# nyu-systems/Grendel-GS

Measured on NVIDIA H100. Metric: train-step Gaussians/s (preprocess+forward+loss+backward), higher is better.
Workload: dtype f32

## Files before the change

### grendel-gs_b200/csrc/loss.cu

```cuda
#include "common.cuh"

#define LS_TILE 32
#define LS_HALO 5
#define LS_IN (LS_TILE + 2 * LS_HALO)
#define LS_THREADS 256

__device__ __constant__ float c_gauss[11];
static unsigned long long g_gauss_ready = 0ull;

static int ensure_gauss() {
    int dev = 0;
    GS_CUDA_TRY(cudaGetDevice(&dev));
    if (dev < 64 && ((g_gauss_ready >> dev) & 1ull)) return GS_OK;
    float g[11], s = 0.f;
    for (int k = 0; k < 11; k++) { g[k] = (float)exp(-((double)(k - 5) * (k - 5)) / (2.0 * 1.5 * 1.5)); s += g[k]; }
    for (int k = 0; k < 11; k++) g[k] = g[k] / s;
    GS_CUDA_TRY(cudaMemcpyToSymbol(c_gauss, g, sizeof(g)));
    if (dev < 64) g_gauss_ready |= 1ull << dev;
    return GS_OK;
}

extern "C" size_t gs_loss_temp_bytes(int rows, int image_width) {
    return (size_t)9 * (size_t)(rows > 0 ? rows : 0) * (size_t)image_width * sizeof(float) + 256;
}

struct LossViews {
    int row0[GS_MAX_VIEWS], rows[GS_MAX_VIEWS];
    int crow0[GS_MAX_VIEWS], crow1[GS_MAX_VIEWS];
    const uint8_t *gt[GS_MAX_VIEWS];
    unsigned long long map_off[GS_MAX_VIEWS];
};

__global__ void __launch_bounds__(LS_THREADS)
k_loss_fwd(int W, int H, const LossViews lv, const float *__restrict__ image, float *__restrict__ maps,
           double *__restrict__ sums) {
    __shared__ float s_x[LS_IN][LS_IN + 1], s_y[LS_IN][LS_IN + 1];
    __shared__ float s_h[5][LS_IN][LS_TILE + 1];
    __shared__ float s_red[2][LS_THREADS / 32];
    const int view = blockIdx.z;
    const int row0 = lv.row0[view], rows = lv.rows[view], crow0 = lv.crow0[view], crow1 = lv.crow1[view];
    const int tx0 = blockIdx.x * LS_TILE, ty0 = blockIdx.y * LS_TILE;
    if (ty0 >= rows) return;
    const size_t HW = (size_t)H * W, SW = (size_t)rows * W;
    const uint8_t *__restrict__ gt = lv.gt[view];
    image += (size_t)view * 3 * HW;
    maps += lv.map_off[view];
    sums += 2 * view;
    const float C1 = 0.01f * 0.01f, C2 = 0.03f * 0.03f;
    float l1 = 0.f, ss = 0.f;
    for (int ch = 0; ch < 3; ch++) {
        for (int k = threadIdx.x; k < LS_IN * LS_IN; k += LS_THREADS) {
            const int r = k / LS_IN, c = k % LS_IN;
            const int y = ty0 + r - LS_HALO, x = tx0 + c - LS_HALO;
            float vx = 0.f, vy = 0.f;
            if (y >= 0 && y < rows && x >= 0 && x < W) {
                vx = image[ch * HW + (size_t)(row0 + y) * W + x];
                vy = fminf(1.f, fmaxf(0.f, (float)gt[ch * SW + (size_t)y * W + x] / 255.0f));
            }
            s_x[r][c] = vx; s_y[r][c] = vy;
        }
        __syncthreads();
        for (int k = threadIdx.x; k < LS_IN * (LS_TILE / 4); k += LS_THREADS) {
            const int r = k / (LS_TILE / 4), c0 = (k % (LS_TILE / 4)) * 4;
            float wx[14], wy[14];
#pragma unroll
            for (int t = 0; t < 14; t++) { wx[t] = s_x[r][c0 + t]; wy[t] = s_y[r][c0 + t]; }
#pragma unroll
            for (int q = 0; q < 4; q++) {
                float a0 = 0.f, a1 = 0.f, a2 = 0.f, a3 = 0.f, a4 = 0.f;
#pragma unroll
                for (int t = 0; t < 11; t++) {
                    const float g = c_gauss[t], vx = wx[q + t], vy = wy[q + t];
                    a0 += g * vx; a1 += g * vy; a2 += g * vx * vx; a3 += g * vy * vy; a4 += g * vx * vy;
                }
                s_h[0][r][c0 + q] = a0; s_h[1][r][c0 + q] = a1; s_h[2][r][c0 + q] = a2; s_h[3][r][c0 + q] = a3;
                s_h[4][r][c0 + q] = a4;
            }
        }
        __syncthreads();
        {
            const int c = threadIdx.x % LS_TILE, r0 = (threadIdx.x / LS_TILE) * 4, x = tx0 + c;
            float m1[4] = {0.f, 0.f, 0.f, 0.f}, m2[4] = {0.f, 0.f, 0.f, 0.f}, e11[4] = {0.f, 0.f, 0.f, 0.f},
                  e22[4] = {0.f, 0.f, 0.f, 0.f}, e12[4] = {0.f, 0.f, 0.f, 0.f};
#pragma unroll
            for (int t = 0; t < 14; t++) {
                const float v0 = s_h[0][r0 + t][c], v1 = s_h[1][r0 + t][c], v2 = s_h[2][r0 + t][c], v3 = s_h[3][r0 + t][c],
                            v4 = s_h[4][r0 + t][c];
#pragma unroll
                for (int q = 0; q < 4; q++) {
                    if (t - q >= 0 && t - q < 11) {
                        const float g = c_gauss[t - q];
                        m1[q] += g * v0; m2[q] += g * v1; e11[q] += g * v2; e22[q] += g * v3; e12[q] += g * v4;
                    }
                }
            }
#pragma unroll
            for (int q = 0; q < 4; q++) {
                const int r = r0 + q, y = ty0 + r;
                if (y < rows && x < W) {
                    const size_t o = (size_t)ch * SW + (size_t)y * W + x;
                    if (y < crow0 || y >= crow1) {
                        maps[o] = 0.f; maps[3 * SW + o] = 0.f; maps[6 * SW + o] = 0.f;
                    } else {
                        const float s1 = e11[q] - m1[q] * m1[q], s2 = e22[q] - m2[q] * m2[q], s12 = e12[q] - m1[q] * m2[q];
                        const float A = 2.f * m1[q] * m2[q] + C1, B = 2.f * s12 + C2,
                                    Cc = m1[q] * m1[q] + m2[q] * m2[q] + C1, D = s1 + s2 + C2;
                        const float iCD = 1.f / (Cc * D);
                        ss += A * B * iCD;
                        const float vx = s_x[r + LS_HALO][c + LS_HALO], vy = s_y[r + LS_HALO][c + LS_HALO];
                        l1 += fabsf(vx - vy);
                        maps[o] = 2.f * m2[q] * (B - A) * iCD - 2.f * m1[q] * A * B * (D - Cc) * iCD * iCD;
                        maps[3 * SW + o] = -A * B * iCD / D;
                        maps[6 * SW + o] = 2.f * A * iCD;
                    }
                }
            }
        }
        __syncthreads();
    }
#pragma unroll
    for (int o = 16; o > 0; o >>= 1) { l1 += __shfl_xor_sync(0xffffffffu, l1, o); ss += __shfl_xor_sync(0xffffffffu, ss, o); }
    if ((threadIdx.x & 31) == 0) { s_red[0][threadIdx.x >> 5] = l1; s_red[1][threadIdx.x >> 5] = ss; }
    __syncthreads();
    if (threadIdx.x == 0) {
        double a = 0.0, b = 0.0;
        for (int w = 0; w < LS_THREADS / 32; w++) { a += (double)s_red[0][w]; b += (double)s_red[1][w]; }
        atomicAdd(&sums[0], a); atomicAdd(&sums[1], b);
    }
}

__global__ void k_loss_finalize(int n, const double *__restrict__ sums, double inv_norm, float *__restrict__ out) {
    const int k = blockIdx.x * blockDim.x + threadIdx.x;
    if (k < 2 * n) out[k] = (float)(sums[k] * inv_norm);
}

__global__ void __launch_bounds__(LS_THREADS)
k_loss_bwd(int W, int H, const LossViews lv, const float *__restrict__ image, const float *__restrict__ maps,
           const float *__restrict__ grad_l1, const float *__restrict__ grad_ssim, float inv_norm,
           float *__restrict__ dimg) {
    __shared__ float s_m[3][LS_IN][LS_IN + 1];
    __shared__ float s_h[3][LS_IN][LS_TILE + 1];
    const int view = blockIdx.z;
    const int row0 = lv.row0[view], rows = lv.rows[view], crow0 = lv.crow0[view], crow1 = lv.crow1[view];
    const int tx0 = blockIdx.x * LS_TILE, ty0 = blockIdx.y * LS_TILE;
    if (ty0 >= rows) return;
    const size_t HW = (size_t)H * W, SW = (size_t)rows * W;
    const uint8_t *__restrict__ gt = lv.gt[view];
    image += (size_t)view * 3 * HW;
    dimg += (size_t)view * 3 * HW;
    maps += lv.map_off[view];
    const float gl1 = grad_l1[view] * inv_norm, gss = grad_ssim[view] * inv_norm;
    for (int ch = 0; ch < 3; ch++) {
        for (int k = threadIdx.x; k < LS_IN * LS_IN; k += LS_THREADS) {
            const int r = k / LS_IN, c = k % LS_IN;
            const int y = ty0 + r - LS_HALO, x = tx0 + c - LS_HALO;
            float v0 = 0.f, v1 = 0.f, v2 = 0.f;
            if (y >= 0 && y < rows && x >= 0 && x < W) {
                const size_t o = (size_t)ch * SW + (size_t)y * W + x;
                v0 = maps[o]; v1 = maps[3 * SW + o]; v2 = maps[6 * SW + o];
            }
            s_m[0][r][c] = v0; s_m[1][r][c] = v1; s_m[2][r][c] = v2;
        }
        __syncthreads();
        for (int k = threadIdx.x; k < LS_IN * (LS_TILE / 4); k += LS_THREADS) {
            const int r = k / (LS_TILE / 4), c0 = (k % (LS_TILE / 4)) * 4;
            float w0[14], w1[14], w2[14];
#pragma unroll
            for (int t = 0; t < 14; t++) { w0[t] = s_m[0][r][c0 + t]; w1[t] = s_m[1][r][c0 + t]; w2[t] = s_m[2][r][c0 + t]; }
#pragma unroll
            for (int q = 0; q < 4; q++) {
                float a0 = 0.f, a1 = 0.f, a2 = 0.f;
#pragma unroll
                for (int t = 0; t < 11; t++) {
                    const float g = c_gauss[t];
                    a0 += g * w0[q + t]; a1 += g * w1[q + t]; a2 += g * w2[q + t];
                }
                s_h[0][r][c0 + q] = a0; s_h[1][r][c0 + q] = a1; s_h[2][r][c0 + q] = a2;
            }
        }
        __syncthreads();
        {
            const int c = threadIdx.x % LS_TILE, r0 = (threadIdx.x / LS_TILE) * 4, x = tx0 + c;
            float b0[4] = {0.f, 0.f, 0.f, 0.f}, b1[4] = {0.f, 0.f, 0.f, 0.f}, b2[4] = {0.f, 0.f, 0.f, 0.f};
#pragma unroll
            for (int t = 0; t < 14; t++) {
                const float v0 = s_h[0][r0 + t][c], v1 = s_h[1][r0 + t][c], v2 = s_h[2][r0 + t][c];
#pragma unroll
                for (int q = 0; q < 4; q++) {
                    if (t - q >= 0 && t - q < 11) {
                        const float g = c_gauss[t - q];
                        b0[q] += g * v0; b1[q] += g * v1; b2[q] += g * v2;
                    }
                }
            }
#pragma unroll
            for (int q = 0; q < 4; q++) {
                const int y = ty0 + r0 + q;
                if (y < rows && x < W) {
                    const size_t oi = ch * HW + (size_t)(row0 + y) * W + x;
                    const float vx = image[oi];
                    const float vy = fminf(1.f, fmaxf(0.f, (float)gt[ch * SW + (size_t)y * W + x] / 255.0f));
                    const float d = vx - vy;
                    const float sgn = (y < crow0 || y >= crow1) ? 0.f : (d > 0.f ? 1.f : (d < 0.f ? -1.f : 0.f));
                    dimg[oi] = gl1 * sgn + gss * (b0[q] + 2.f * vx * b1[q] + vy * b2[q]);
                }
            }
        }
        __syncthreads();
    }
}

#define LS_HEADER_1 ((size_t)256)
#define LS_HEADER_B ((size_t)(2 * sizeof(double) * GS_MAX_VIEWS))

static int make_loss_views(int num_views, int H, int W, const int32_t *rows4, const void *const *gts, LossViews &lv,
                           int *max_rows, size_t *sum_rows) {
    GS_REQUIRE(num_views >= 1 && num_views <= GS_MAX_VIEWS, "num_views must be in [1, GS_MAX_VIEWS]");
    GS_REQUIRE(H > 0 && W > 0 && rows4 && gts, "sizes");
    size_t off = 0;
    int mx = 0;
    for (int v = 0; v < GS_MAX_VIEWS; v++) {
        lv.row0[v] = lv.rows[v] = lv.crow0[v] = lv.crow1[v] = 0;
        lv.gt[v] = nullptr;
        lv.map_off[v] = 0ull;
        if (v >= num_views) continue;
        const int row0 = rows4[4 * v], row1 = rows4[4 * v + 1], c0 = rows4[4 * v + 2], c1 = rows4[4 * v + 3];
        const int rows = row1 - row0;
        GS_REQUIRE(row0 >= 0 && row1 <= H && rows >= 0, "strip rows");
        if (rows == 0) continue;
        GS_REQUIRE(c0 >= row0 && c1 <= row1 && c1 >= c0, "count rows must lie inside [row0,row1)");
        GS_REQUIRE(gts[v] != nullptr, "null ground-truth pointer");
        lv.row0[v] = row0; lv.rows[v] = rows; lv.crow0[v] = c0 - row0; lv.crow1[v] = c1 - row0;
        lv.gt[v] = (const uint8_t *)gts[v];
        lv.map_off[v] = (unsigned long long)off;
        off += (size_t)9 * rows * W;
        mx = rows > mx ? rows : mx;
    }
    *max_rows = mx;
    *sum_rows = off / ((size_t)9 * W);
    return GS_OK;
}

static int loss_forward_impl(int num_views, int H, int W, const int32_t *rows4, const float *image, const void *const *gts,
                             float *out, void *temp, size_t temp_bytes, size_t header, cudaStream_t stream) {
    GS_REQUIRE(image && out && temp, "null pointer");
    LossViews lv;
    int max_rows = 0;
    size_t sum_rows = 0;
    int rc = make_loss_views(num_views, H, W, rows4, gts, lv, &max_rows, &sum_rows);
    if (rc != GS_OK) return rc;
    if (temp_bytes < header + (size_t)9 * sum_rows * W * sizeof(float)) {
        gs_set_error("gs_loss_forward: temp too small");
        return GS_ENOMEM;
    }
    rc = ensure_gauss();
    if (rc != GS_OK) return rc;
    double *sums = (double *)temp;
    float *maps = (float *)((char *)temp + header);
    GS_CUDA_TRY(cudaMemsetAsync(sums, 0, 2 * sizeof(double) * (size_t)num_views, stream));
    GsStageTimer timer(GS_STAGE_LOSS_FWD, stream);
    if (max_rows > 0) {
        dim3 grid((W + LS_TILE - 1) / LS_TILE, (max_rows + LS_TILE - 1) / LS_TILE, num_views);
        k_loss_fwd<<<grid, LS_THREADS, 0, stream>>>(W, H, lv, image, maps, sums);
        GS_LAUNCH_CHECK();
    }
    k_loss_finalize<<<1, 2 * GS_MAX_VIEWS, 0, stream>>>(num_views, sums, 1.0 / (3.0 * (double)H * (double)W), out);
    GS_LAUNCH_CHECK();
    return GS_OK;
}

static int loss_backward_impl(int num_views, int H, int W, const int32_t *rows4, const float *image,
                              const void *const *gts, const void *temp, const float *grad_l1, const float *grad_ssim,
                              float *dimg, size_t header, cudaStream_t stream) {
    GS_REQUIRE(image && temp && grad_l1 && grad_ssim && dimg, "null pointer");
    LossViews lv;
    int max_rows = 0;
    size_t sum_rows = 0;
    int rc = make_loss_views(num_views, H, W, rows4, gts, lv, &max_rows, &sum_rows);
    if (rc != GS_OK) return rc;
    rc = ensure_gauss();
    if (rc != GS_OK) return rc;
    const float *maps = (const float *)((const char *)temp + header);
    const size_t HW = (size_t)H * W;
    if (num_views == 1) {
        const int row0 = lv.row0[0], row1 = lv.row0[0] + lv.rows[0];
        for (int ch = 0; ch < 3; ch++) {
            if (row0 > 0) GS_CUDA_TRY(cudaMemsetAsync(dimg + ch * HW, 0, sizeof(float) * (size_t)row0 * W, stream));
            if (row1 < H)
                GS_CUDA_TRY(cudaMemsetAsync(dimg + ch * HW + (size_t)row1 * W, 0, sizeof(float) * (size_t)(H - row1) * W, stream));
        }
    } else if (sum_rows < (size_t)num_views * H) {
        GS_CUDA_TRY(cudaMemsetAsync(dimg, 0, sizeof(float) * 3 * HW * (size_t)num_views, stream));
    }
    if (max_rows == 0) return GS_OK;
    dim3 grid((W + LS_TILE - 1) / LS_TILE, (max_rows + LS_TILE - 1) / LS_TILE, num_views);
    GsStageTimer timer(GS_STAGE_LOSS_BWD, stream);
    k_loss_bwd<<<grid, LS_THREADS, 0, stream>>>(W, H, lv, image, maps, grad_l1, grad_ssim,
                                                (float)(1.0 / (3.0 * (double)H * (double)W)), dimg);
    GS_LAUNCH_CHECK();
    return GS_OK;
}

extern "C" int gs_loss_forward(int image_height, int image_width, int row0, int row1, int count_row0, int count_row1,
                               const float *image, const uint8_t *gt_u8, float *out_l1_ssim, void *temp,
                               size_t temp_bytes, void *stream_) {
    GS_REQUIRE(row1 > row0, "strip rows");
    GS_REQUIRE(gt_u8, "null pointer");
    const int32_t rows4[4] = {row0, row1, count_row0, count_row1};
    const void *gts[1] = {gt_u8};
    return loss_forward_impl(1, image_height, image_width, rows4, image, gts, out_l1_ssim, temp, temp_bytes, LS_HEADER_1,
                             (cudaStream_t)stream_);
}

extern "C" size_t gs_loss_temp_bytes_batched(int num_views, const int32_t *rows4_host, int image_width) {
    size_t rows = 0;
    for (int v = 0; v < num_views && rows4_host; v++) {
        const int r = rows4_host[4 * v + 1] - rows4_host[4 * v];
        rows += r > 0 ? (size_t)r : 0;
    }
    return LS_HEADER_B + (size_t)9 * rows * (size_t)(image_width > 0 ? image_width : 0) * sizeof(float) + 256;
}

extern "C" int gs_loss_forward_batched(int num_views, int image_height, int image_width, const int32_t *rows4_host,
                                       const float *image, const void *const *gt_u8_ptrs_host, float *out_l1_ssim,
                                       void *temp, size_t temp_bytes, void *stream_) {
    return loss_forward_impl(num_views, image_height, image_width, rows4_host, image, gt_u8_ptrs_host, out_l1_ssim, temp,
                             temp_bytes, LS_HEADER_B, (cudaStream_t)stream_);
}

extern "C" int gs_loss_backward(int image_height, int image_width, int row0, int row1, int count_row0, int count_row1,
                                const float *image, const uint8_t *gt_u8, const void *temp, const float *grad_l1,
                                const float *grad_ssim, float *dL_dimage, void *stream_) {
    GS_REQUIRE(row1 > row0, "strip rows");
    GS_REQUIRE(gt_u8, "null pointer");
    const int32_t rows4[4] = {row0, row1, count_row0, count_row1};
    const void *gts[1] = {gt_u8};
    return loss_backward_impl(1, image_height, image_width, rows4, image, gts, temp, grad_l1, grad_ssim, dL_dimage,
                              LS_HEADER_1, (cudaStream_t)stream_);
}

extern "C" int gs_loss_backward_batched(int num_views, int image_height, int image_width, const int32_t *rows4_host,
                                        const float *image, const void *const *gt_u8_ptrs_host, const void *temp,
                                        const float *grad_l1, const float *grad_ssim, float *dL_dimage, void *stream_) {
    return loss_backward_impl(num_views, image_height, image_width, rows4_host, image, gt_u8_ptrs_host, temp, grad_l1,
                              grad_ssim, dL_dimage, LS_HEADER_B, (cudaStream_t)stream_);
}
```

Baseline: 597.0 million.

## Restructure SSIM loss kernels into per-channel vertical strips with ring-buffered halo reuse

The forward and backward SSIM/L1 loss kernels now give each CTA one channel and a strip of up to 96 rows instead of a 32x32 tile over all three channels. Row-filtered results sit in a shared-memory ring buffer, so vertical halo rows are reused across consecutive 32-row chunks rather than recomputed per tile. Global loads for the next chunk are software-prefetched into registers while the current chunk is filtered. Blocks shrink to 128 threads with a minimum-CTA launch bound, and the row pass uses float4 shared accesses. The aim is less redundant halo loading and filtering plus better latency hiding, at the cost of more registers, fewer CTAs, and a more complex schedule. A separate profiling script times the loss kernels.

```diff
diff --git a/grendel-gs_b200/csrc/loss.cu b/grendel-gs_b200/csrc/loss.cu
--- a/grendel-gs_b200/csrc/loss.cu
+++ b/grendel-gs_b200/csrc/loss.cu
@@ -1,9 +1,15 @@
 #include "common.cuh"
 
-#define LS_TILE 32
 #define LS_HALO 5
-#define LS_IN (LS_TILE + 2 * LS_HALO)
-#define LS_THREADS 256
+#define LS_TW 32
+#define LS_IW (LS_TW + 2 * LS_HALO)
+#define LS_SP 44
+#define LS_CR 32
+#define LS_RING (LS_CR + 2 * LS_HALO)
+#define LS_STRIP (3 * LS_CR)
+#define LS_THREADS 128
+#define LS_MIN_CTAS 5
+#define LS_VR (LS_CR / (LS_THREADS / 32))
 
 __device__ __constant__ float c_gauss[11];
 static unsigned long long g_gauss_ready = 0ull;
@@ -31,101 +37,193 @@
     unsigned long long map_off[GS_MAX_VIEWS];
 };
 
-__global__ void __launch_bounds__(LS_THREADS)
+GS_D float gt_value(uint32_t v) {
+    const float f = (float)v, r = 1.0f / 255.0f;
+    const float q = __fmul_rn(f, r);
+    return __fmaf_rn(__fmaf_rn(-q, 255.0f, f), r, q);
+}
+
+#define LS_SSLOTS ((LS_CR * LS_IW + LS_THREADS - 1) / LS_THREADS)
+GS_D bool stage_slot(int m, int n, int &r, int &c) {
+    const int e = threadIdx.x + m * LS_THREADS;
+    r = e / LS_IW;
+    c = e - r * LS_IW;
+    return r < n;
+}
+
+template <int NI, int NQ>
+GS_D void row_pass(const float (*s_in)[LS_CR][LS_SP], float (*s_h)[LS_RING][LS_TW], int i0, int n) {
+    for (int k = threadIdx.x; k < n * (LS_TW / 4); k += LS_THREADS) {
+        const int r = k / (LS_TW / 4), c0 = (k % (LS_TW / 4)) * 4;
+        float w[NI][16];
+#pragma unroll
+        for (int p = 0; p < NI; p++)
+#pragma unroll
+            for (int m = 0; m < 4; m++) {
+                const float4 v = *reinterpret_cast<const float4 *>(&s_in[p][r][c0 + 4 * m]);
+                w[p][4 * m] = v.x; w[p][4 * m + 1] = v.y; w[p][4 * m + 2] = v.z; w[p][4 * m + 3] = v.w;
+            }
+        float a[NQ][4];
+#pragma unroll
+        for (int p = 0; p < NQ; p++)
+#pragma unroll
+            for (int q = 0; q < 4; q++) a[p][q] = 0.f;
+#pragma unroll
+        for (int j = 0; j < 14; j++) {
+            float v[NQ];
+#pragma unroll
+            for (int p = 0; p < NI; p++) v[p] = w[p][j];
+            if (NI == 2) { v[2] = w[0][j] * w[0][j]; v[3] = w[1][j] * w[1][j]; v[4] = w[0][j] * w[1][j]; }
+#pragma unroll
+            for (int q = 0; q < 4; q++) {
+                const int t = j - q;
+                if (t >= 0 && t < 11) {
+#pragma unroll
+                    for (int p = 0; p < NQ; p++) a[p][q] = fmaf(c_gauss[t], v[p], a[p][q]);
+                }
+            }
+        }
+        const int slot = (i0 + r) % LS_RING;
+#pragma unroll
+        for (int p = 0; p < NQ; p++)
+            *reinterpret_cast<float4 *>(&s_h[p][slot][c0]) = make_float4(a[p][0], a[p][1], a[p][2], a[p][3]);
+    }
+}
+
+template <int NQ>
+GS_D void col_pass(const float (*s_h)[LS_RING][LS_TW], int o0, float (&a)[NQ][LS_VR]) {
+    const int c = threadIdx.x % LS_TW;
+    int slot = (o0 + (threadIdx.x / 32) * LS_VR) % LS_RING;
+#pragma unroll
+    for (int p = 0; p < NQ; p++)
+#pragma unroll
+        for (int q = 0; q < LS_VR; q++) a[p][q] = 0.f;
+#pragma unroll
+    for (int j = 0; j < LS_VR + 10; j++) {
+        float v[NQ];
+#pragma unroll
+        for (int p = 0; p < NQ; p++) v[p] = s_h[p][slot][c];
+#pragma unroll
+        for (int q = 0; q < LS_VR; q++) {
+            const int t = j - q;
+            if (t >= 0 && t < 11) {
+#pragma unroll
+                for (int p = 0; p < NQ; p++) a[p][q] = fmaf(c_gauss[t], v[p], a[p][q]);
+            }
+        }
+        slot = slot == LS_RING - 1 ? 0 : slot + 1;
+    }
+}
+
+struct StripCta {
+    int view, ch, rows, sy0, span, tx0;
+    GS_D StripCta(const LossViews &lv) {
+        view = blockIdx.z;
+        ch = blockIdx.y % 3;
+        rows = lv.rows[view];
+        sy0 = (blockIdx.y / 3) * LS_STRIP;
+        span = min(LS_STRIP, rows - sy0);
+        tx0 = blockIdx.x * LS_TW;
+    }
+};
+
+template <class Load, class Store, class Row, class Col>
+GS_D void strip_schedule(int span, Load &&load, Store &&store, Row &&row, Col &&col) {
+    const int units = 1 + (span + LS_CR - 1) / LS_CR;
+    auto first = [](int u) { return u == 0 ? 0 : 2 * LS_HALO + (u - 1) * LS_CR; };
+    auto count = [span](int u) { return u == 0 ? 2 * LS_HALO : min(LS_CR, span - (u - 1) * LS_CR); };
+    load(first(0), count(0));
+    store(first(0), count(0));
+    __syncthreads();
+    for (int u = 0; u < units; u++) {
+        if (u + 1 < units) load(first(u + 1), count(u + 1));
+        row(first(u), count(u));
+        __syncthreads();
+        if (u + 1 < units) store(first(u + 1), count(u + 1));
+        if (u > 0) col((u - 1) * LS_CR, count(u));
+        __syncthreads();
+    }
+}
+
+__global__ void __launch_bounds__(LS_THREADS, LS_MIN_CTAS)
 k_loss_fwd(int W, int H, const LossViews lv, const float *__restrict__ image, float *__restrict__ maps,
            double *__restrict__ sums) {
-    __shared__ float s_x[LS_IN][LS_IN + 1], s_y[LS_IN][LS_IN + 1];
-    __shared__ float s_h[5][LS_IN][LS_TILE + 1];
+    __shared__ __align__(16) float s_in[2][LS_CR][LS_SP];
+    __shared__ __align__(16) float s_h[5][LS_RING][LS_TW];
     __shared__ float s_red[2][LS_THREADS / 32];
-    const int view = blockIdx.z;
-    const int row0 = lv.row0[view], rows = lv.rows[view], crow0 = lv.crow0[view], crow1 = lv.crow1[view];
-    const int tx0 = blockIdx.x * LS_TILE, ty0 = blockIdx.y * LS_TILE;
-    if (ty0 >= rows) return;
+    const StripCta b(lv);
+    if (b.span <= 0) return;
+    const int rows = b.rows, crow0 = max(lv.crow0[b.view], b.sy0), crow1 = min(lv.crow1[b.view], b.sy0 + b.span);
     const size_t HW = (size_t)H * W, SW = (size_t)rows * W;
-    const uint8_t *__restrict__ gt = lv.gt[view];
-    image += (size_t)view * 3 * HW;
-    maps += lv.map_off[view];
-    sums += 2 * view;
+    const float *__restrict__ xin = image + ((size_t)b.view * 3 + b.ch) * HW + (size_t)lv.row0[b.view] * W;
+    const uint8_t *__restrict__ yin = lv.gt[b.view] + b.ch * SW;
+    maps += lv.map_off[b.view] + b.ch * SW;
+    const int lane = threadIdx.x % 32, warp = threadIdx.x / 32, x = b.tx0 + lane;
     const float C1 = 0.01f * 0.01f, C2 = 0.03f * 0.03f;
     float l1 = 0.f, ss = 0.f;
-    for (int ch = 0; ch < 3; ch++) {
-        for (int k = threadIdx.x; k < LS_IN * LS_IN; k += LS_THREADS) {
-            const int r = k / LS_IN, c = k % LS_IN;
-            const int y = ty0 + r - LS_HALO, x = tx0 + c - LS_HALO;
-            float vx = 0.f, vy = 0.f;
-            if (y >= 0 && y < rows && x >= 0 && x < W) {
-                vx = image[ch * HW + (size_t)(row0 + y) * W + x];
-                vy = fminf(1.f, fmaxf(0.f, (float)gt[ch * SW + (size_t)y * W + x] / 255.0f));
-            }
-            s_x[r][c] = vx; s_y[r][c] = vy;
-        }
-        __syncthreads();
-        for (int k = threadIdx.x; k < LS_IN * (LS_TILE / 4); k += LS_THREADS) {
-            const int r = k / (LS_TILE / 4), c0 = (k % (LS_TILE / 4)) * 4;
-            float wx[14], wy[14];
-#pragma unroll
-            for (int t = 0; t < 14; t++) { wx[t] = s_x[r][c0 + t]; wy[t] = s_y[r][c0 + t]; }
-#pragma unroll
-            for (int q = 0; q < 4; q++) {
-                float a0 = 0.f, a1 = 0.f, a2 = 0.f, a3 = 0.f, a4 = 0.f;
-#pragma unroll
-                for (int t = 0; t < 11; t++) {
-                    const float g = c_gauss[t], vx = wx[q + t], vy = wy[q + t];
-                    a0 += g * vx; a1 += g * vy; a2 += g * vx * vx; a3 += g * vy * vy; a4 += g * vx * vy;
+    float vx[LS_SSLOTS];
+    uint32_t vg[LS_SSLOTS];
+    auto load = [&](int i0, int n) {
+        const int y0 = b.sy0 - LS_HALO + i0;
+        const ptrdiff_t base = (ptrdiff_t)y0 * W + (b.tx0 - LS_HALO);
+#pragma unroll
+        for (int m = 0; m < LS_SSLOTS; m++) {
+            int r, c;
+            const bool slot = stage_slot(m, n, r, c);
+            vx[m] = 0.f; vg[m] = 0u;
+            if (slot && (unsigned)(y0 + r) < (unsigned)rows && (unsigned)(b.tx0 - LS_HALO + c) < (unsigned)W) {
+                vx[m] = xin[base + r * W + c];
+                vg[m] = yin[base + r * W + c];
+            }
+        }
+    };
+    auto store = [&](int i0, int n) {
+#pragma unroll
+        for (int m = 0; m < LS_SSLOTS; m++) {
+            int r, c;
+            if (!stage_slot(m, n, r, c)) continue;
+            const float vy = gt_value(vg[m]);
+            if ((unsigned)(b.sy0 - LS_HALO + i0 + r - crow0) < (unsigned)(crow1 - crow0) &&
+                (unsigned)(c - LS_HALO) < (unsigned)min(LS_TW, W - b.tx0))
+                l1 += fabsf(vx[m] - vy);
+            s_in[0][r][c] = vx[m]; s_in[1][r][c] = vy;
+        }
+    };
+    auto row = [&](int i0, int n) { row_pass<2, 5>(s_in, s_h, i0, n); };
+    auto col = [&](int o0, int n) {
+        float a[5][LS_VR];
+        col_pass<5>(s_h, o0, a);
+        const int yb = b.sy0 + o0 + warp * LS_VR;
+        float *mp = maps + (ptrdiff_t)yb * W + x;
+#pragma unroll
+        for (int q = 0; q < LS_VR; q++) {
+            const int y = yb + q;
+            if (warp * LS_VR + q < n && x < W) {
+                const int off = q * W;
+                if (y < crow0 || y >= crow1) {
+                    mp[off] = 0.f; mp[3 * SW + off] = 0.f; mp[6 * SW + off] = 0.f;
+                } else {
+                    const float m1 = a[0][q], m2 = a[1][q];
+                    const float s1 = a[2][q] - m1 * m1, s2 = a[3][q] - m2 * m2, s12 = a[4][q] - m1 * m2;
+                    const float A = 2.f * m1 * m2 + C1, B = 2.f * s12 + C2, Cc = m1 * m1 + m2 * m2 + C1, D = s1 + s2 + C2;
+                    const float iCD = 1.f / (Cc * D);
+                    ss += A * B * iCD;
+                    mp[off] = 2.f * m2 * (B - A) * iCD - 2.f * m1 * A * B * (D - Cc) * iCD * iCD;
+                    mp[3 * SW + off] = -A * B * iCD / D;
+                    mp[6 * SW + off] = 2.f * A * iCD;
                 }
-                s_h[0][r][c0 + q] = a0; s_h[1][r][c0 + q] = a1; s_h[2][r][c0 + q] = a2; s_h[3][r][c0 + q] = a3;
-                s_h[4][r][c0 + q] = a4;
-            }
-        }
-        __syncthreads();
-        {
-            const int c = threadIdx.x % LS_TILE, r0 = (threadIdx.x / LS_TILE) * 4, x = tx0 + c;
-            float m1[4] = {0.f, 0.f, 0.f, 0.f}, m2[4] = {0.f, 0.f, 0.f, 0.f}, e11[4] = {0.f, 0.f, 0.f, 0.f},
-                  e22[4] = {0.f, 0.f, 0.f, 0.f}, e12[4] = {0.f, 0.f, 0.f, 0.f};
-#pragma unroll
-            for (int t = 0; t < 14; t++) {
-                const float v0 = s_h[0][r0 + t][c], v1 = s_h[1][r0 + t][c], v2 = s_h[2][r0 + t][c], v3 = s_h[3][r0 + t][c],
-                            v4 = s_h[4][r0 + t][c];
-#pragma unroll
-                for (int q = 0; q < 4; q++) {
-                    if (t - q >= 0 && t - q < 11) {
-                        const float g = c_gauss[t - q];
-                        m1[q] += g * v0; m2[q] += g * v1; e11[q] += g * v2; e22[q] += g * v3; e12[q] += g * v4;
-                    }
-                }
-            }
-#pragma unroll
-            for (int q = 0; q < 4; q++) {
-                const int r = r0 + q, y = ty0 + r;
-                if (y < rows && x < W) {
-                    const size_t o = (size_t)ch * SW + (size_t)y * W + x;
-                    if (y < crow0 || y >= crow1) {
-                        maps[o] = 0.f; maps[3 * SW + o] = 0.f; maps[6 * SW + o] = 0.f;
-                    } else {
-                        const float s1 = e11[q] - m1[q] * m1[q], s2 = e22[q] - m2[q] * m2[q], s12 = e12[q] - m1[q] * m2[q];
-                        const float A = 2.f * m1[q] * m2[q] + C1, B = 2.f * s12 + C2,
-                                    Cc = m1[q] * m1[q] + m2[q] * m2[q] + C1, D = s1 + s2 + C2;
-                        const float iCD = 1.f / (Cc * D);
-                        ss += A * B * iCD;
-                        const float vx = s_x[r + LS_HALO][c + LS_HALO], vy = s_y[r + LS_HALO][c + LS_HALO];
-                        l1 += fabsf(vx - vy);
-                        maps[o] = 2.f * m2[q] * (B - A) * iCD - 2.f * m1[q] * A * B * (D - Cc) * iCD * iCD;
-                        maps[3 * SW + o] = -A * B * iCD / D;
-                        maps[6 * SW + o] = 2.f * A * iCD;
-                    }
-                }
-            }
-        }
-        __syncthreads();
-    }
+            }
+        }
+    };
+    strip_schedule(b.span, load, store, row, col);
 #pragma unroll
     for (int o = 16; o > 0; o >>= 1) { l1 += __shfl_xor_sync(0xffffffffu, l1, o); ss += __shfl_xor_sync(0xffffffffu, ss, o); }
-    if ((threadIdx.x & 31) == 0) { s_red[0][threadIdx.x >> 5] = l1; s_red[1][threadIdx.x >> 5] = ss; }
+    if (lane == 0) { s_red[0][warp] = l1; s_red[1][warp] = ss; }
     __syncthreads();
     if (threadIdx.x == 0) {
-        double a = 0.0, b = 0.0;
-        for (int w = 0; w < LS_THREADS / 32; w++) { a += (double)s_red[0][w]; b += (double)s_red[1][w]; }
-        atomicAdd(&sums[0], a); atomicAdd(&sums[1], b);
+        double a = 0.0, c = 0.0;
+        for (int w = 0; w < LS_THREADS / 32; w++) { a += (double)s_red[0][w]; c += (double)s_red[1][w]; }
+        atomicAdd(&sums[2 * b.view], a); atomicAdd(&sums[2 * b.view + 1], c);
     }
 }
 
@@ -134,80 +232,69 @@
     if (k < 2 * n) out[k] = (float)(sums[k] * inv_norm);
 }
 
-__global__ void __launch_bounds__(LS_THREADS)
+__global__ void __launch_bounds__(LS_THREADS, LS_MIN_CTAS)
 k_loss_bwd(int W, int H, const LossViews lv, const float *__restrict__ image, const float *__restrict__ maps,
            const float *__restrict__ grad_l1, const float *__restrict__ grad_ssim, float inv_norm,
            float *__restrict__ dimg) {
-    __shared__ float s_m[3][LS_IN][LS_IN + 1];
-    __shared__ float s_h[3][LS_IN][LS_TILE + 1];
-    const int view = blockIdx.z;
-    const int row0 = lv.row0[view], rows = lv.rows[view], crow0 = lv.crow0[view], crow1 = lv.crow1[view];
-    const int tx0 = blockIdx.x * LS_TILE, ty0 = blockIdx.y * LS_TILE;
-    if (ty0 >= rows) return;
+    __shared__ __align__(16) float s_in[3][LS_CR][LS_SP];
+    __shared__ __align__(16) float s_h[3][LS_RING][LS_TW];
+    const StripCta b(lv);
+    if (b.span <= 0) return;
+    const int rows = b.rows, crow0 = lv.crow0[b.view], crow1 = lv.crow1[b.view];
     const size_t HW = (size_t)H * W, SW = (size_t)rows * W;
-    const uint8_t *__restrict__ gt = lv.gt[view];
-    image += (size_t)view * 3 * HW;
-    dimg += (size_t)view * 3 * HW;
-    maps += lv.map_off[view];
-    const float gl1 = grad_l1[view] * inv_norm, gss = grad_ssim[view] * inv_norm;
-    for (int ch = 0; ch < 3; ch++) {
-        for (int k = threadIdx.x; k < LS_IN * LS_IN; k += LS_THREADS) {
-            const int r = k / LS_IN, c = k % LS_IN;
-            const int y = ty0 + r - LS_HALO, x = tx0 + c - LS_HALO;
-            float v0 = 0.f, v1 = 0.f, v2 = 0.f;
-            if (y >= 0 && y < rows && x >= 0 && x < W) {
-                const size_t o = (size_t)ch * SW + (size_t)y * W + x;
-                v0 = maps[o]; v1 = maps[3 * SW + o]; v2 = maps[6 * SW + o];
-            }
-            s_m[0][r][c] = v0; s_m[1][r][c] = v1; s_m[2][r][c] = v2;
-        }
-        __syncthreads();
-        for (int k = threadIdx.x; k < LS_IN * (LS_TILE / 4); k += LS_THREADS) {
-            const int r = k / (LS_TILE / 4), c0 = (k % (LS_TILE / 4)) * 4;
-            float w0[14], w1[14], w2[14];
-#pragma unroll
-            for (int t = 0; t < 14; t++) { w0[t] = s_m[0][r][c0 + t]; w1[t] = s_m[1][r][c0 + t]; w2[t] = s_m[2][r][c0 + t]; }
-#pragma unroll
-            for (int q = 0; q < 4; q++) {
-                float a0 = 0.f, a1 = 0.f, a2 = 0.f;
-#pragma unroll
-                for (int t = 0; t < 11; t++) {
-                    const float g = c_gauss[t];
-                    a0 += g * w0[q + t]; a1 += g * w1[q + t]; a2 += g * w2[q + t];
-                }
-                s_h[0][r][c0 + q] = a0; s_h[1][r][c0 + q] = a1; s_h[2][r][c0 + q] = a2;
-            }
-        }
-        __syncthreads();
-        {
-            const int c = threadIdx.x % LS_TILE, r0 = (threadIdx.x / LS_TILE) * 4, x = tx0 + c;
-            float b0[4] = {0.f, 0.f, 0.f, 0.f}, b1[4] = {0.f, 0.f, 0.f, 0.f}, b2[4] = {0.f, 0.f, 0.f, 0.f};
-#pragma unroll
-            for (int t = 0; t < 14; t++) {
-                const float v0 = s_h[0][r0 + t][c], v1 = s_h[1][r0 + t][c], v2 = s_h[2][r0 + t][c];
-#pragma unroll
-                for (int q = 0; q < 4; q++) {
-                    if (t - q >= 0 && t - q < 11) {
-                        const float g = c_gauss[t - q];
-                        b0[q] += g * v0; b1[q] += g * v1; b2[q] += g * v2;
-                    }
-                }
-            }
-#pragma unroll
-            for (int q = 0; q < 4; q++) {
-                const int y = ty0 + r0 + q;
-                if (y < rows && x < W) {
-                    const size_t oi = ch * HW + (size_t)(row0 + y) * W + x;
-                    const float vx = image[oi];
-                    const float vy = fminf(1.f, fmaxf(0.f, (float)gt[ch * SW + (size_t)y * W + x] / 255.0f));
-                    const float d = vx - vy;
-                    const float sgn = (y < crow0 || y >= crow1) ? 0.f : (d > 0.f ? 1.f : (d < 0.f ? -1.f : 0.f));
-                    dimg[oi] = gl1 * sgn + gss * (b0[q] + 2.f * vx * b1[q] + vy * b2[q]);
-                }
-            }
-        }
-        __syncthreads();
-    }
+    const size_t plane = ((size_t)b.view * 3 + b.ch) * HW + (size_t)lv.row0[b.view] * W;
+    const float *__restrict__ xin = image + plane;
+    const uint8_t *__restrict__ yin = lv.gt[b.view] + b.ch * SW;
+    dimg += plane;
+    maps += lv.map_off[b.view] + b.ch * SW;
+    const int warp = threadIdx.x / 32, x = b.tx0 + threadIdx.x % 32;
+    const float gl1 = grad_l1[b.view] * inv_norm, gss = grad_ssim[b.view] * inv_norm;
+    float v[LS_SSLOTS][3];
+    auto load = [&](int i0, int n) {
+        const int y0 = b.sy0 - LS_HALO + i0;
+        const float *mp = maps + (ptrdiff_t)y0 * W + (b.tx0 - LS_HALO);
+#pragma unroll
+        for (int m = 0; m < LS_SSLOTS; m++) {
+            int r, c;
+            const bool slot = stage_slot(m, n, r, c);
+            v[m][0] = v[m][1] = v[m][2] = 0.f;
+            if (slot && (unsigned)(y0 + r) < (unsigned)rows && (unsigned)(b.tx0 - LS_HALO + c) < (unsigned)W) {
+                const int off = r * W + c;
+                v[m][0] = mp[off]; v[m][1] = mp[3 * SW + off]; v[m][2] = mp[6 * SW + off];
+            }
+        }
+    };
+    auto store = [&](int, int n) {
+#pragma unroll
+        for (int m = 0; m < LS_SSLOTS; m++) {
+            int r, c;
+            if (!stage_slot(m, n, r, c)) continue;
+            s_in[0][r][c] = v[m][0]; s_in[1][r][c] = v[m][1]; s_in[2][r][c] = v[m][2];
+        }
+    };
+    auto row = [&](int i0, int n) { row_pass<3, 3>(s_in, s_h, i0, n); };
+    auto col = [&](int o0, int n) {
+        const int yb = b.sy0 + o0 + warp * LS_VR;
+        const ptrdiff_t pb = (ptrdiff_t)yb * W + x;
+        float px[LS_VR], py[LS_VR];
+#pragma unroll
+        for (int q = 0; q < LS_VR; q++) {
+            px[q] = py[q] = 0.f;
+            if (warp * LS_VR + q < n && x < W) { px[q] = xin[pb + q * W]; py[q] = gt_value(yin[pb + q * W]); }
+        }
+        float a[3][LS_VR];
+        col_pass<3>(s_h, o0, a);
+#pragma unroll
+        for (int q = 0; q < LS_VR; q++) {
+            const int y = yb + q;
+            if (warp * LS_VR + q < n && x < W) {
+                const float d = px[q] - py[q];
+                const float sgn = (y < crow0 || y >= crow1) ? 0.f : (d > 0.f ? 1.f : (d < 0.f ? -1.f : 0.f));
+                dimg[pb + q * W] = gl1 * sgn + gss * (a[0][q] + 2.f * px[q] * a[1][q] + py[q] * a[2][q]);
+            }
+        }
+    };
+    strip_schedule(b.span, load, store, row, col);
 }
 
 #define LS_HEADER_1 ((size_t)256)
@@ -241,6 +328,10 @@
     return GS_OK;
 }
 
+static dim3 loss_grid(int W, int max_rows, int num_views) {
+    return dim3((W + LS_TW - 1) / LS_TW, 3 * ((max_rows + LS_STRIP - 1) / LS_STRIP), num_views);
+}
+
 static int loss_forward_impl(int num_views, int H, int W, const int32_t *rows4, const float *image, const void *const *gts,
                              float *out, void *temp, size_t temp_bytes, size_t header, cudaStream_t stream) {
     GS_REQUIRE(image && out && temp, "null pointer");
@@ -260,8 +351,7 @@
     GS_CUDA_TRY(cudaMemsetAsync(sums, 0, 2 * sizeof(double) * (size_t)num_views, stream));
     GsStageTimer timer(GS_STAGE_LOSS_FWD, stream);
     if (max_rows > 0) {
-        dim3 grid((W + LS_TILE - 1) / LS_TILE, (max_rows + LS_TILE - 1) / LS_TILE, num_views);
-        k_loss_fwd<<<grid, LS_THREADS, 0, stream>>>(W, H, lv, image, maps, sums);
+        k_loss_fwd<<<loss_grid(W, max_rows, num_views), LS_THREADS, 0, stream>>>(W, H, lv, image, maps, sums);
         GS_LAUNCH_CHECK();
     }
     k_loss_finalize<<<1, 2 * GS_MAX_VIEWS, 0, stream>>>(num_views, sums, 1.0 / (3.0 * (double)H * (double)W), out);
@@ -293,10 +383,9 @@
         GS_CUDA_TRY(cudaMemsetAsync(dimg, 0, sizeof(float) * 3 * HW * (size_t)num_views, stream));
     }
     if (max_rows == 0) return GS_OK;
-    dim3 grid((W + LS_TILE - 1) / LS_TILE, (max_rows + LS_TILE - 1) / LS_TILE, num_views);
     GsStageTimer timer(GS_STAGE_LOSS_BWD, stream);
-    k_loss_bwd<<<grid, LS_THREADS, 0, stream>>>(W, H, lv, image, maps, grad_l1, grad_ssim,
-                                                (float)(1.0 / (3.0 * (double)H * (double)W)), dimg);
+    k_loss_bwd<<<loss_grid(W, max_rows, num_views), LS_THREADS, 0, stream>>>(
+        W, H, lv, image, maps, grad_l1, grad_ssim, (float)(1.0 / (3.0 * (double)H * (double)W)), dimg);
     GS_LAUNCH_CHECK();
     return GS_OK;
 }
diff --git a/profiles/time_loss.py b/profiles/time_loss.py
--- /dev/null
+++ b/profiles/time_loss.py
@@ -0,0 +1,109 @@
+#!/usr/bin/env python
+import argparse
+import json
+import os
+import subprocess
+import sys
+
+ROOT = os.path.dirname(os.path.dirname(os.path.abspath(__file__)))
+for _p in (ROOT, os.path.join(ROOT, "grendel-gs_b200")):
+    if _p not in sys.path:
+        sys.path.insert(0, _p)
+
+FWD_BYTES, BWD_BYTES = 51, 63
+
+
+def card():
+    import torch
+    out = {"name": torch.cuda.get_device_name(0), "power_limit_w": None, "sm_clock_max_mhz": None}
+    try:
+        r = subprocess.run(["nvidia-smi", "--id=0", "--query-gpu=power.limit,clocks.max.sm", "--format=csv,noheader,nounits"],
+                           capture_output=True, text=True, timeout=30)
+        p, c = (v.strip() for v in r.stdout.strip().split(","))
+        out["power_limit_w"], out["sm_clock_max_mhz"] = float(p), float(c)
+    except Exception:
+        pass
+    return out
+
+
+def time_calls(fn, launches, warmup):
+    import torch
+    for _ in range(warmup):
+        fn()
+    torch.cuda.synchronize()
+    a, b = torch.cuda.Event(enable_timing=True), torch.cuda.Event(enable_timing=True)
+    a.record()
+    for _ in range(launches):
+        fn()
+    b.record()
+    torch.cuda.synchronize()
+    return a.elapsed_time(b) * 1e3 / launches
+
+
+def measure(H, W, rows4, launches, warmup):
+    import torch
+    from gs_b200 import _lib
+    row0, row1, c0, c1 = rows4
+    rows = row1 - row0
+    g = torch.Generator(device="cuda").manual_seed(0)
+    image = torch.rand((3, H, W), generator=g, device="cuda", dtype=torch.float32)
+    gt = torch.randint(0, 256, (3, rows, W), generator=g, device="cuda", dtype=torch.uint8)
+    tb = _lib.query("gs_loss_temp_bytes", rows, W)
+    temp = torch.empty((tb,), dtype=torch.uint8, device="cuda")
+    out = torch.empty((2,), dtype=torch.float32, device="cuda")
+    gw = torch.tensor([0.8, -0.2], dtype=torch.float32, device="cuda")
+    dimg = torch.empty_like(image)
+    s = torch.cuda.current_stream().cuda_stream
+
+    def fwd():
+        _lib.call("gs_loss_forward", H, W, row0, row1, c0, c1, image.data_ptr(), gt.data_ptr(), out.data_ptr(),
+                  temp.data_ptr(), tb, s)
+
+    def bwd():
+        _lib.call("gs_loss_backward", H, W, row0, row1, c0, c1, image.data_ptr(), gt.data_ptr(), temp.data_ptr(),
+                  gw.data_ptr(), gw.data_ptr() + 4, dimg.data_ptr(), s)
+
+    fwd()
+    res = {"shape": f"{W}x{H}", "rows": [row0, row1], "count_rows": [c0, c1], "launches": launches, "warmup": warmup}
+    for name, fn, per_px in (("forward", fwd, FWD_BYTES), ("backward", bwd, BWD_BYTES)):
+        us = time_calls(fn, launches, warmup)
+        _lib.profile_enable(True)
+        for _ in range(launches):
+            fn()
+        torch.cuda.synchronize()
+        stages = _lib.profile_read()
+        _lib.profile_enable(False)
+        st = stages.get("loss " + name)
+        kernel_us = st[0] * 1e3 / st[1] if st else None
+        nbytes = per_px * rows * W
+        res[name] = {"us_per_call": round(us, 2), "us_stage_timer": None if kernel_us is None else round(kernel_us, 2),
+                     "compulsory_bytes": nbytes, "gbs_per_call": round(nbytes / (us * 1e-6) / 1e9, 1),
+                     "frac_of_3350_gbs": round(nbytes / (us * 1e-6) / 3350e9, 3)}
+    res["loss"] = [float(v) for v in out.cpu()]
+    return res
+
+
+def main():
+    ap = argparse.ArgumentParser(description=__doc__.splitlines()[0])
+    ap.add_argument("--launches", type=int, default=400)
+    ap.add_argument("--warmup", type=int, default=20)
+    ap.add_argument("--out", default=os.path.join(ROOT, "runs", "time_loss.json"))
+    args = ap.parse_args()
+    import torch
+    if not torch.cuda.is_available():
+        raise SystemExit("time_loss.py needs a CUDA device")
+    from gs_b200 import _lib
+    _lib.load()
+    H, W = 1080, 1920
+    q = H // 4
+    result = {"library": _lib.LIB_PATH, "gpu": card(),
+              "full": measure(H, W, (0, H, 0, H), args.launches, args.warmup),
+              "strip": measure(H, W, (q - 5, 2 * q + 5, q, 2 * q), args.launches, args.warmup)}
+    os.makedirs(os.path.dirname(os.path.abspath(args.out)), exist_ok=True)
+    with open(args.out, "w") as f:
+        json.dump(result, f, indent=1)
+    print(json.dumps(result), flush=True)
+
+
+if __name__ == "__main__":
+    main()
```

Result: faster. 607.5 million, median of 6 (+1.7%).
